# hangxu0304/DeepReduce

Measured on NVIDIA H100. Metric: ResNet-50 images/sec (whole job, device-timed, max over ranks), higher is better.
Workload: dtype bf16

## Files before the change

deepreduce_b200/ops/csrc/bn.cu:

```cuda
#include <cuda_bf16.h>

#include <algorithm>

#include "common.cuh"
#include "ops.h"

namespace dr {

namespace {

constexpr int kVec = 8;
constexpr int kApplyThreads = 256;
constexpr int kReduceThreads = 128;

struct ChanParams {
  float m[kVec], inv[kVec], w[kVec], b[kVec];
};

__device__ __forceinline__ void load8(const float* __restrict__ p, float* d) {
  const float4 a = __ldg(reinterpret_cast<const float4*>(p));
  const float4 b = __ldg(reinterpret_cast<const float4*>(p) + 1);
  d[0] = a.x; d[1] = a.y; d[2] = a.z; d[3] = a.w;
  d[4] = b.x; d[5] = b.y; d[6] = b.z; d[7] = b.w;
}
// ... 145 lines not shown
  q.sh = h - 2 * ph + 1;
  q.sw = w - 2 * pw + 1;
  q.off = ((n * pg.Ho + ph) * pg.Wo + pw) * C + c;
#pragma unroll
  for (int k = 0; k < 4; ++k) {
    const int a = k >> 1, b = k & 1;
    q.code[k] = a < q.nh && b < q.nw ? *reinterpret_cast<const uint2*>(codes + q.off + (a * pg.Wo + b) * C) : uint2{};
  }
}

template <bool kTwo>
__device__ __forceinline__ void pool_gather_grads(PoolGather& q, const __nv_bfloat16* __restrict__ gp,
                                                  const __nv_bfloat16* __restrict__ gp2, const PoolGeom& pg, int C) {
#pragma unroll
  for (int k = 0; k < 4; ++k) {
    const int a = k >> 1, b = k & 1;
    const bool in = a < q.nh && b < q.nw;
    const int off = q.off + (a * pg.Wo + b) * C;
    q.g[k] = in ? *reinterpret_cast<const uint4*>(gp + off) : uint4{};
    if (kTwo && in) q.g[k] = add_bf16x8(q.g[k], *reinterpret_cast<const uint4*>(gp2 + off));
  }
}

__device__ __forceinline__ void pool_gather_resolve(const PoolGather& q, uint4& g, unsigned& bits) {
  __nv_bfloat16* hg = reinterpret_cast<__nv_bfloat16*>(&g);
  const bool single = q.nh == 1 && q.nw == 1;
  bits = 0;
#pragma unroll
  for (int i = 0; i < kVec; ++i) {
    float s = 0.f;
    __nv_bfloat16 one = __float2bfloat16_rn(0.f);
    unsigned bit = 0;
#pragma unroll
    for (int k = 0; k < 4; ++k) {
      const int a = k >> 1, b = k & 1;
      const unsigned code = (reinterpret_cast<const uint8_t*>(&q.code[k]))[i];
      if (a < q.nh && b < q.nw && (int)(code & 0x7fu) == (q.sh - 2 * a) * 3 + (q.sw - 2 * b)) {
        const __nv_bfloat16 v = (reinterpret_cast<const __nv_bfloat16*>(&q.g[k]))[i];
        s = __fadd_rn(s, __bfloat162float(v));
        one = v;
        bit = code >> 7;
      }
    }
    hg[i] = single ? one : __float2bfloat16_rn(s);
    bits |= bit << i;
  }
}

template <bool kTwo>
__global__ void __launch_bounds__(kApplyThreads) bn_pool_grad_kernel(const __nv_bfloat16* __restrict__ gp,
                                                                     const __nv_bfloat16* __restrict__ gp2,
                                                                     const uint8_t* __restrict__ codes,
                                                                     __nv_bfloat16* __restrict__ g, PoolGeom pg,
                                                                     int64_t rows, int C) {
  const int groups = C / kVec;
  const int rows_per_cta = blockDim.x / groups;
  const int rsub = threadIdx.x / groups;
  if (rsub >= rows_per_cta) return;
  const int c = (threadIdx.x % groups) * kVec;
  const int64_t step = (int64_t)gridDim.x * rows_per_cta;
#pragma unroll 2
  for (int64_t r = (int64_t)blockIdx.x * rows_per_cta + rsub; r < rows; r += step) {
    PoolGather q;
    pool_gather_codes(q, codes, pg, (int)r, C, c, true);
    pool_gather_grads<kTwo>(q, gp, gp2, pg, C);
    uint4 v;
    unsigned bits;
    pool_gather_resolve(q, v, bits);
    __nv_bfloat16* hv = reinterpret_cast<__nv_bfloat16*>(&v);
#pragma unroll
    for (int i = 0; i < kVec; ++i)
      if (!((bits >> i) & 1u)) hv[i] = __float2bfloat16_rn(0.f);
    *reinterpret_cast<uint4*>(g + r * C + c) = v;
  }
}

struct RowTree {
  int block_y, grid_y;
  __host__ __device__ int S() const { return block_y * grid_y; }
  __host__ __device__ int loops(int rows) const { return 1 + (rows - 1) / (S() * kLoads); }
  static constexpr int kLoads = 4;
};

constexpr int kStatsThreads = 256;

__device__ __forceinline__ void welford_update(float x, float inv, float valid, float& mean, float& m2n) {
  const float d0 = __fsub_rn(x, mean);
  mean = __fmaf_rn(d0, inv, mean);
  const float d1 = __fsub_rn(x, mean);
  m2n = __fmaf_rn(__fmul_rn(d0, d1), valid, m2n);
}

template <int kN, bool kFuseNew>
__device__ __forceinline__ void welford_merge(int& n, float* mean, float* m2n, int n_new, const float* mean_new,
                                              const float* m2n_new) {
  const float fn = (float)n, fn_new = (float)n_new;
  const float factor = __frcp_rn((float)max(1, n + n_new));
#pragma unroll
  for (int i = 0; i < kN; ++i) {
    const float d = __fsub_rn(mean[i], mean_new[i]);
    const float s = kFuseNew ? __fmaf_rn(mean_new[i], fn_new, __fmul_rn(mean[i], fn))
                             : __fmaf_rn(mean[i], fn, __fmul_rn(mean_new[i], fn_new));
    mean[i] = __fmul_rn(s, factor);
    const float u = __fmul_rn(__fmul_rn(__fmul_rn(d, d), fn_new), fn);
    m2n[i] = __fadd_rn(m2n[i], __fmaf_rn(u, factor, m2n_new[i]));
  }
  n += n_new;
}

template <int kN>
struct WelfordSlots {
  float* mean; float* m2n; int* count;
  __device__ WelfordSlots(float* sh, int slots)
      : mean(sh), m2n(sh + slots * kN), count(reinterpret_cast<int*>(sh + 2 * slots * kN)) {}
  __device__ void put(int s, int n, const float* m, const float* q) const {
#pragma unroll
    for (int i = 0; i < kN; ++i) { mean[s * kN + i] = m[i]; m2n[s * kN + i] = q[i]; }
    count[s] = n;
  }
  template <bool kFuseNew>
  __device__ void merge_from(int s, int& n, float* m, float* q) const {
    float mn[kN], qn[kN];
#pragma unroll
    for (int i = 0; i < kN; ++i) { mn[i] = mean[s * kN + i]; qn[i] = m2n[s * kN + i]; }
    welford_merge<kN, kFuseNew>(n, m, q, count[s], mn, qn);
  }
  static size_t bytes(int slots) { return (size_t)slots * (2 * kN * sizeof(float) + sizeof(int)); }
};

template <int kN>
__device__ __forceinline__ void welford_tree_over_y(const WelfordSlots<kN>& sl, bool part, int y, int block_y, int base,
                                                    int stride, int& n, float* mean, float* m2n) {
  for (int off = block_y / 2; off > 0; off >>= 1) {
    if (part && y < 2 * off) sl.put(base + y * stride, n, mean, m2n);
    __syncthreads();
    if (part && y < off) sl.template merge_from<false>(base + (y + off) * stride, n, mean, m2n);
    __syncthreads();
  }
}

struct StatsOut {
  float* mean; float* invstd; float* running_mean; float* running_var;
  float* st_mean; float* st_m2n; int* st_count;
  float momentum, bessel, eps;
};

__device__ __forceinline__ void stats_store(const StatsOut& o, int c, int n, float mean, float m2n) {
  const float var = __fdiv_rn(m2n, (float)n);
  const float keep = __fsub_rn(1.f, o.momentum);
  o.mean[c] = mean;
  o.invstd[c] = rsqrtf(__fadd_rn(var, o.eps));
  o.running_mean[c] = __fmaf_rn(mean, o.momentum, __fmul_rn(o.running_mean[c], keep));
  o.running_var[c] = __fmaf_rn(__fmul_rn(var, o.bessel), o.momentum, __fmul_rn(o.running_var[c], keep));
}

__global__ void __launch_bounds__(kStatsThreads) bn_stats_kernel(const __nv_bfloat16* __restrict__ x, StatsOut o,
                                                                 RowTree t, int rows, int C) {
  constexpr int L = RowTree::kLoads;
  constexpr int kAhead = 4;
  extern __shared__ float sh[];
  const int gpc = blockDim.x / (L * t.block_y);
  const int g = threadIdx.x % gpc, j = (threadIdx.x / gpc) % L, y = threadIdx.x / (gpc * L);
  const int group = blockIdx.x * gpc + g;
  const bool live = group * kVec < C;
  const int c = live ? group * kVec : 0;
  const int S = t.S();
  const int n_loops = t.loops(rows);
  const int r0 = blockIdx.y * t.block_y + y + j * S;
  const int rstep = L * S;
  float mean[kVec], m2n[kVec];
#pragma unroll
  for (int i = 0; i < kVec; ++i) mean[i] = m2n[i] = 0.f;
  int n = 0;
  auto load = [&](uint4* b, int i0) {
#pragma unroll
    for (int u = 0; u < kAhead; ++u) {
      const int r = r0 + (i0 + u) * rstep;
      b[u] = live && i0 + u < n_loops && r < rows ? *reinterpret_cast<const uint4*>(x + (size_t)r * C + c) : uint4{};
    }
  };
  uint4 cur[kAhead];
  load(cur, 0);
  for (int i0 = 0; i0 < n_loops; i0 += kAhead) {
    uint4 nxt[kAhead];
    load(nxt, i0 + kAhead);
#pragma unroll
    for (int u = 0; u < kAhead; ++u) {
      const int i = i0 + u;
      if (i >= n_loops) break;
      const bool valid = r0 + i * rstep < rows;
      const float inv = valid ? __frcp_rn((float)(i + 1)) : 0.f;
      const float fv = valid ? 1.f : 0.f;
      n += valid;
      const __nv_bfloat16* hx = reinterpret_cast<const __nv_bfloat16*>(&cur[u]);
#pragma unroll
      for (int k = 0; k < kVec; ++k) welford_update(__bfloat162float(hx[k]), inv, fv, mean[k], m2n[k]);
    }
#pragma unroll
    for (int u = 0; u < kAhead; ++u) cur[u] = nxt[u];
  }
  const WelfordSlots<kVec> sl(sh, blockDim.x);
  sl.put(threadIdx.x, n, mean, m2n);
  __syncthreads();
  if (j == 0) {
#pragma unroll
    for (int a = 1; a < L; ++a) sl.merge_from<true>(threadIdx.x + a * gpc, n, mean, m2n);
  }
  __syncthreads();
  welford_tree_over_y<kVec>(sl, j == 0, y, t.block_y, g, gpc * L, n, mean, m2n);
  if (j != 0 || y != 0 || !live) return;
  if (t.grid_y == 1) {
#pragma unroll
    for (int i = 0; i < kVec; ++i) stats_store(o, c + i, n, mean[i], m2n[i]);
    return;
  }
#pragma unroll
  for (int i = 0; i < kVec; ++i) {
    o.st_mean[(size_t)blockIdx.y * C + c + i] = mean[i];
    o.st_m2n[(size_t)blockIdx.y * C + c + i] = m2n[i];
  }
  if (group == 0) o.st_count[blockIdx.y] = n;
}

__global__ void bn_stats_finalize_kernel(StatsOut o, RowTree t, int C) {
  extern __shared__ float sh[];
  const int cols = blockDim.x / t.block_y;
  const int col = threadIdx.x % cols, y = threadIdx.x / cols;
  const int c = blockIdx.x * cols + col;
  int n = 0;
  float mean = 0.f, m2n = 0.f;
  if (c < C)
    for (int b = y; b < t.grid_y; b += t.block_y) {
      const float mb = o.st_mean[(size_t)b * C + c], qb = o.st_m2n[(size_t)b * C + c];
      welford_merge<1, false>(n, &mean, &m2n, o.st_count[b], &mb, &qb);
    }
  const WelfordSlots<1> sl(sh, blockDim.x);
  welford_tree_over_y<1>(sl, true, y, t.block_y, col, cols, n, &mean, &m2n);
  if (y == 0 && c < C) stats_store(o, c, n, mean, m2n);
}


template <int kN>
__device__ __forceinline__ void tree_over_y(float* v, float* sh, int y, int n, int col, int width) {
  for (int off = n / 2; off > 0; off >>= 1) {
#pragma unroll
    for (int i = 0; i < kN; ++i) sh[y * width + col + i] = v[i];
    __syncthreads();
    if (y < off) {
#pragma unroll
      for (int i = 0; i < kN; ++i) v[i] = __fadd_rn(v[i], sh[(y + off) * width + col + i]);
    }
    __syncthreads();
  }
}

struct BwdOut {
  float* sums;
  float* dw; float* db; float* dwz; float* dbz;
  float* staging;
};

__device__ __forceinline__ void bwd_store(const BwdOut& o, int k, int c, int C, float v, const float* invstd,
                                         const float* invstd_z) {
  o.sums[k * C + c] = v;
  if (k == 0) {
    o.db[c] = v;
    if (o.dbz) o.dbz[c] = v;
  } else if (k == 1) {
    o.dw[c] = __fmul_rn(v, invstd[c]);
  } else {
    o.dwz[c] = __fmul_rn(v, invstd_z[c]);
  }
}

__device__ __forceinline__ float masked(__nv_bfloat16 go, unsigned bit) { return bit ? __bfloat162float(go) : 0.f; }

template <int kMode, bool kTwo>
__global__ void __launch_bounds__(kReduceThreads) bn_bwd_reduce_kernel(const __nv_bfloat16* __restrict__ go,
                                                                       const __nv_bfloat16* __restrict__ go2,
                                                                       const uint8_t* __restrict__ mask,
                                                                       const __nv_bfloat16* __restrict__ x,
                                                                       const float* __restrict__ mean,
                                                                       const float* __restrict__ invstd,
                                                                       const __nv_bfloat16* __restrict__ z,
                                                                       const float* __restrict__ mean_z,
                                                                       const float* __restrict__ invstd_z,
                                                                       __nv_bfloat16* __restrict__ g_out, BwdOut o,
                                                                       RowTree t, int rows, int C) {
  constexpr int kSums = kMode == 2 ? 3 : 2;
  constexpr int L = RowTree::kLoads;
  extern __shared__ float sh[];
  const int gpc = blockDim.x / t.block_y;
  const int tg = threadIdx.x % gpc, y = threadIdx.x / gpc;
  const int group = blockIdx.x * gpc + tg;
  const bool live = group * kVec < C;
  const int c = live ? group * kVec : 0;
  const int S = t.S();
  float m[kVec], mz[kVec];
#pragma unroll
  for (int i = 0; i < kVec; ++i) {
    m[i] = mean[c + i];
    mz[i] = kMode == 2 ? mean_z[c + i] : 0.f;
  }
  float acc[kSums][L][kVec];
#pragma unroll
  for (int k = 0; k < kSums; ++k)
#pragma unroll
    for (int j = 0; j < L; ++j)
#pragma unroll
      for (int i = 0; i < kVec; ++i) acc[k][j][i] = 0.f;
  const int mgroups = C / kVec;
  int r = blockIdx.y * t.block_y + y;
  const int n_loops = t.loops(rows);
  constexpr bool kAhead = !(kTwo && kMode == 2);
  struct Batch {
    uint4 g[L], g2[L], x[L], z[L];
    unsigned m[L];
  };
  auto load = [&](Batch& b, int r0) {
#pragma unroll
    for (int j = 0; j < L; ++j) {
// ... 186 lines not shown
  bn_apply_kernel<kMode><<<grid, threads, 0, st>>>(reinterpret_cast<const __nv_bfloat16*>(x), px,
                                                   reinterpret_cast<const __nv_bfloat16*>(z), pz,
                                                   reinterpret_cast<__nv_bfloat16*>(out),
                                                   reinterpret_cast<uint8_t*>(mask), rows, C);
  return cudaGetLastError();
}

int last_pow2(unsigned n) {
  n |= n >> 1; n |= n >> 2; n |= n >> 4; n |= n >> 8; n |= n >> 16;
  return std::max<int>(1, (int)(n - (n >> 1)));
}

RowTree row_tree(int rows, int C) {
  const int block_x = std::min(last_pow2((unsigned)C), 32);
  const int block_y = std::min(last_pow2((unsigned)((rows + 15) / 16)), 512 / block_x);
  int grid_y = std::min((rows + block_y * 16 - 1) / (block_y * 16), 128);
  if (grid_y < 8) grid_y = 1;
  return {block_y, grid_y};
}

template <int kMode, bool kTwo>
cudaError_t launch_bwd_reduce(const BnBwd& b, const RowTree& t, const BwdOut& o, int rows, int C, cudaStream_t st) {
  const int groups = C / kVec;
  const int gpc = std::min(groups, std::max(1, kReduceThreads / t.block_y));
  const dim3 grid((groups + gpc - 1) / gpc, t.grid_y);
  const int threads = gpc * t.block_y;
  count_launch();
  bn_bwd_reduce_kernel<kMode, kTwo><<<grid, threads, threads * kVec * sizeof(float), st>>>(
      reinterpret_cast<const __nv_bfloat16*>(b.go), reinterpret_cast<const __nv_bfloat16*>(b.go2), b.mask,
      reinterpret_cast<const __nv_bfloat16*>(b.x), b.px.mean, b.px.invstd, reinterpret_cast<const __nv_bfloat16*>(b.z),
      b.pz.mean, b.pz.invstd, reinterpret_cast<__nv_bfloat16*>(b.g), o, t, rows, C);
  return cudaGetLastError();
}

template <int kMode, bool kTwo>
cudaError_t launch_bwd_elemt(const BnBwd& b, const ElemtArgs& a, int64_t rows, int C, cudaStream_t st) {
  int grid = 0, threads = 0;
  cudaError_t e = rows_grid(bn_bwd_elemt_kernel<kMode, kTwo>, rows, C, grid, threads);
  if (e != cudaSuccess) return e;
  const float norm = (float)(1.0 / (double)rows);
  count_launch();
  bn_bwd_elemt_kernel<kMode, kTwo><<<grid, threads, 0, st>>>(
      reinterpret_cast<const __nv_bfloat16*>(kMode == 1 || kMode == 3 ? b.g : b.go),
      reinterpret_cast<const __nv_bfloat16*>(b.go2), b.mask, reinterpret_cast<const __nv_bfloat16*>(b.x),
      reinterpret_cast<const __nv_bfloat16*>(b.z), a, reinterpret_cast<__nv_bfloat16*>(b.dx),
      reinterpret_cast<__nv_bfloat16*>(b.dz), norm, rows, C);
  return cudaGetLastError();
}

template <int kMode, bool kTwo>
cudaError_t launch_backward(const BnBwd& b, int64_t rows64, int C, cudaStream_t st) {
  const int rows = (int)rows64;
  const RowTree t = row_tree(rows, C);
  const BwdOut o{b.sums, b.dw, b.db, b.dwz, b.dbz, b.staging};
  cudaError_t e;
  if (kMode == 3) {
    int grid = 0, threads = 0;
    e = rows_grid(bn_pool_grad_kernel<kTwo>, rows64, C, grid, threads);
    if (e != cudaSuccess) return e;
    count_launch();
    bn_pool_grad_kernel<kTwo><<<grid, threads, 0, st>>>(reinterpret_cast<const __nv_bfloat16*>(b.go),
                                                        reinterpret_cast<const __nv_bfloat16*>(b.go2), b.mask,
                                                        reinterpret_cast<__nv_bfloat16*>(b.g), b.pool, rows64, C);
    e = cudaGetLastError();
    if (e != cudaSuccess) return e;
  }
  BnBwd bb = b;
  if (kMode == 3) bb.go = b.g;
  e = launch_bwd_reduce<kMode, kTwo && kMode != 3>(bb, t, o, rows, C, st);
  if (e != cudaSuccess) return e;
  if (t.grid_y > 1) {
    const int cols = std::max(1, 512 / t.block_y);
    const int threads = cols * t.block_y;
    count_launch();
    bn_bwd_finalize_kernel<<<(C + cols - 1) / cols, threads, threads * sizeof(float), st>>>(
        o, t, kMode == 2 ? 3 : 2, C, b.px.invstd, b.pz.invstd);
    e = cudaGetLastError();
    if (e != cudaSuccess) return e;
  }
  const ElemtArgs a{b.px.mean, b.px.invstd, b.px.weight, b.sums, b.pz.mean, b.pz.invstd, b.pz.weight};
  return launch_bwd_elemt<kMode, kTwo && kMode == 2>(b, a, rows64, C, st);
}

cudaError_t launch_stats(const BnStats& s, int rows, int C, cudaStream_t st) {
  const RowTree t = row_tree(rows, C);
  const int grid_y = t.grid_y;
  const StatsOut o{s.mean, s.invstd, s.running_mean, s.running_var,
                   s.staging, s.staging + (size_t)grid_y * C, reinterpret_cast<int*>(s.staging + 2 * (size_t)grid_y * C),
                   s.momentum, s.bessel, s.eps};
  const int groups = C / kVec;
  const int gpc = std::min(groups, std::max(1, kStatsThreads / (RowTree::kLoads * t.block_y)));
  const int threads = gpc * RowTree::kLoads * t.block_y;
  count_launch();
  bn_stats_kernel<<<dim3((groups + gpc - 1) / gpc, grid_y), threads, WelfordSlots<kVec>::bytes(threads), st>>>(
      reinterpret_cast<const __nv_bfloat16*>(s.x), o, t, rows, C);
  cudaError_t e = cudaGetLastError();
  if (e != cudaSuccess || grid_y == 1) return e;
  const int cols = std::max(1, 512 / t.block_y);
  const int fthreads = cols * t.block_y;
  count_launch();
  bn_stats_finalize_kernel<<<(C + cols - 1) / cols, fthreads, WelfordSlots<1>::bytes(fthreads), st>>>(o, t, C);
  return cudaGetLastError();
}

}

void bn_row_tree(int64_t rows, int C, int* block_y, int* grid_y) {
  const RowTree t = row_tree((int)rows, C);
  *block_y = t.block_y;
  *grid_y = t.grid_y;
}

cudaError_t launch_bn_backward(int mode, const BnBwd& b, int64_t rows, int C, cudaStream_t st) {
  if (rows == 0) return cudaSuccess;
  const bool two = b.go2 != nullptr;
  switch (mode) {
    case 0: return two ? cudaErrorInvalidValue : launch_backward<0, false>(b, rows, C, st);
    case 1: return two ? launch_backward<1, true>(b, rows, C, st) : launch_backward<1, false>(b, rows, C, st);
    case 2: return two ? launch_backward<2, true>(b, rows, C, st) : launch_backward<2, false>(b, rows, C, st);
    case 3: return two ? launch_backward<3, true>(b, rows, C, st) : launch_backward<3, false>(b, rows, C, st);
    default: return cudaErrorInvalidValue;
  }
}

cudaError_t launch_bn_stats(const BnStats& s, int64_t rows, int C, cudaStream_t st) {
  if (rows == 0) return cudaSuccess;
  return launch_stats(s, (int)rows, C, st);
}

cudaError_t launch_bn_update_stats(const float* mean, float* var_invstd, float* running_mean, float* running_var, int C,
                                   float momentum, float bessel, float eps, cudaStream_t st) {
  count_launch();
  bn_update_stats_kernel<<<(C + 255) / 256, 256, 0, st>>>(mean, var_invstd, running_mean, running_var, C, momentum,
                                                          bessel, eps);
  return cudaGetLastError();
}

cudaError_t launch_bn_apply(int mode, const void* x, const BnParams& px, const void* z, const BnParams& pz, void* out,
                            void* mask, int64_t rows, int C, cudaStream_t st) {
  switch (mode) {
    case 0: return launch_apply<0>(x, px, z, pz, out, mask, rows, C, st);
    case 1: return launch_apply<1>(x, px, z, pz, out, mask, rows, C, st);
    case 2: return launch_apply<2>(x, px, z, pz, out, mask, rows, C, st);
    default: return cudaErrorInvalidValue;
  }
}

cudaError_t launch_bn_apply_pool(const void* x, const BnParams& px, void* out, void* codes, int N, const PoolGeom& pg,
                                 int C, cudaStream_t st) {
  const int64_t orows = (int64_t)N * pg.Ho * pg.Wo;
  if (orows == 0) return cudaSuccess;
  int grid = 0, threads = 0;
  cudaError_t e = rows_grid(bn_apply_pool_kernel, orows, C, grid, threads);
  if (e != cudaSuccess) return e;
  count_launch();
  bn_apply_pool_kernel<<<grid, threads, 0, st>>>(reinterpret_cast<const __nv_bfloat16*>(x), px,
                                                 reinterpret_cast<__nv_bfloat16*>(out),
                                                 reinterpret_cast<uint8_t*>(codes), orows, pg, C);
  return cudaGetLastError();
}

}
```

deepreduce_b200/ops/csrc/binding.cpp:

```cpp
#include <ATen/cuda/CUDAContext.h>
#include <c10/cuda/CUDAGuard.h>
#include <c10/cuda/CUDAStream.h>
#include <torch/extension.h>

#include <algorithm>
#include <condition_variable>
#include <deque>
#include <mutex>
#include <thread>

#include "ops.h"

namespace py = pybind11;
using dr::EngineParams;

#define CHECK_CUDA_T(x) TORCH_CHECK((x).is_cuda() && (x).is_contiguous(), #x " must be a contiguous CUDA tensor")

static cudaStream_t cur_stream() { return at::cuda::getCurrentCUDAStream().stream(); }

static void check_last(const char* what) {
  cudaError_t e = cudaGetLastError();
  TORCH_CHECK(e == cudaSuccess, what, ": ", cudaGetErrorString(e));
}

// ... 237 lines not shown
                  ") lies outside the DDP buffer of ", ddp_numel, " elements");
      TORCH_CHECK(e >= 0 && e % V == 0, "Repack: segment ", i, " starts at engine element ", e,
                  ", not on a 16-byte vector");
      TORCH_CHECK((e + n + V - 1) / V * V <= eng_numel, "Repack: segment ", i, " [", e, ", ", e + n,
                  ") lies outside the engine buffer of ", eng_numel, " elements");
      h[4 * i] = d; h[4 * i + 1] = e; h[4 * i + 2] = n; h[4 * i + 3] = n_vec;
      n_vec += (n + V - 1) / V;
      ddp_ranges.emplace_back(d, d + n);
      eng_ranges.emplace_back(e, e + n);
    }
    h[4 * n_seg] = 0; h[4 * n_seg + 1] = 0; h[4 * n_seg + 2] = 0; h[4 * n_seg + 3] = n_vec;
    for (auto* r : {&ddp_ranges, &eng_ranges}) {
      std::sort(r->begin(), r->end());
      for (size_t i = 1; i < r->size(); ++i)
        TORCH_CHECK((*r)[i].first >= (*r)[i - 1].second, "Repack: segments overlap at element ", (*r)[i].first);
    }
    table = host.to(device);
  }

  void check_buffers(const torch::Tensor& ddp, const torch::Tensor& eng) const {
    for (const torch::Tensor* t : {&ddp, &eng}) {
      TORCH_CHECK(t->is_cuda() && t->is_contiguous() && t->dim() == 1, "Repack: buffers are contiguous 1-D CUDA tensors");
      TORCH_CHECK(t->scalar_type() == dtype, "Repack: the table was built for ", dtype, " buffers, got ", t->scalar_type());
      TORCH_CHECK(t->device() == table.device(), "Repack: buffer on ", t->device(), ", table on ", table.device());
    }
    TORCH_CHECK(ddp.numel() >= ddp_numel, "Repack: the DDP buffer has ", ddp.numel(), " elements, the table needs ", ddp_numel);
    TORCH_CHECK(eng.numel() >= eng_numel, "Repack: the engine buffer has ", eng.numel(), " elements, the table needs ", eng_numel);
    TORCH_CHECK(reinterpret_cast<uintptr_t>(eng.data_ptr()) % 16 == 0, "Repack: the engine buffer must be 16-byte aligned");
  }

  void pack(torch::Tensor ddp, torch::Tensor eng) const {
    check_buffers(ddp, eng);
    c10::cuda::CUDAGuard g(eng.device());
    cudaError_t e = dr::launch_bucket_repack(true, elem_bytes, ddp.data_ptr(), eng.data_ptr(), table.data_ptr<int64_t>(),
                                             (int)n_seg, n_vec, cur_stream());
    TORCH_CHECK(e == cudaSuccess, "bucket_pack: ", cudaGetErrorString(e));
  }

  void unpack(torch::Tensor eng, torch::Tensor ddp) const {
    check_buffers(ddp, eng);
    c10::cuda::CUDAGuard g(eng.device());
    cudaError_t e = dr::launch_bucket_repack(false, elem_bytes, eng.data_ptr(), ddp.data_ptr(), table.data_ptr<int64_t>(),
                                             (int)n_seg, n_vec, cur_stream());
    TORCH_CHECK(e == cudaSuccess, "bucket_unpack: ", cudaGetErrorString(e));
  }
};

namespace at::native {
struct Var;
template <typename scalar_t, typename VarTransform>
void batch_norm_stats_channels_last_cuda_template(const at::Tensor& out_mean, const at::Tensor& out_invstd,
                                                   const at::Tensor& input, double epsilon);
}

static void check_bn_input(const torch::Tensor& x) {
  TORCH_CHECK(x.is_cuda() && x.scalar_type() == torch::kBFloat16 && x.dim() == 4 && x.stride(1) == 1 &&
                  x.is_contiguous(at::MemoryFormat::ChannelsLast),
              "bn: x must be a channels_last bf16 CUDA tensor");
  TORCH_CHECK(x.size(1) % 8 == 0 && x.size(1) <= 8192, "bn: channels must be a multiple of 8, at most 8192");
  TORCH_CHECK(x.numel() < std::numeric_limits<int32_t>::max(), "bn: tensor too large for 32-bit indexing");
}

static void check_chan(const torch::Tensor& t, int64_t C, const char* what) {
  TORCH_CHECK(t.is_cuda() && t.scalar_type() == torch::kFloat32 && t.is_contiguous() && t.numel() == C, "bn: ", what,
              " must be a contiguous float32 CUDA tensor of C elements");
}

static std::vector<torch::Tensor> bn_stats(torch::Tensor x, torch::Tensor running_mean, torch::Tensor running_var,
                                           double momentum, double eps, bool torch_kernel) {
  check_bn_input(x);
  const int64_t C = x.size(1);
  check_chan(running_mean, C, "running_mean");
  check_chan(running_var, C, "running_var");
  const int64_t N = x.numel() / C;
  TORCH_CHECK(N > 1, "bn: expected more than 1 value per channel when training");
  c10::cuda::CUDAGuard g(x.device());
  auto opts = x.options().dtype(torch::kFloat32);
  auto mean = torch::empty({C}, opts), invstd = torch::empty({C}, opts);
  const float bessel = static_cast<float>(static_cast<double>(N) / static_cast<double>(N - 1));
  int block_y = 0, grid_y = 0;
  dr::bn_row_tree(N, (int)C, &block_y, &grid_y);
  cudaError_t e;
  if (!torch_kernel && (int64_t)block_y * grid_y <= N) {
    auto staging = grid_y > 1 ? torch::empty({(2 * C + 1) * grid_y}, opts) : torch::Tensor();
    const dr::BnStats s{x.data_ptr(), mean.data_ptr<float>(), invstd.data_ptr<float>(), running_mean.data_ptr<float>(),
                        running_var.data_ptr<float>(), grid_y > 1 ? staging.data_ptr<float>() : nullptr,
                        (float)momentum, bessel, (float)eps};
    e = dr::launch_bn_stats(s, N, (int)C, cur_stream());
  } else {
    at::native::batch_norm_stats_channels_last_cuda_template<c10::BFloat16, at::native::Var>(mean, invstd, x, eps);
    e = dr::launch_bn_update_stats(mean.data_ptr<float>(), invstd.data_ptr<float>(), running_mean.data_ptr<float>(),
                                   running_var.data_ptr<float>(), (int)C, (float)momentum, bessel, (float)eps,
                                   cur_stream());
  }
  TORCH_CHECK(e == cudaSuccess, "bn_stats: ", cudaGetErrorString(e));
  return {mean, invstd};
}

static dr::BnParams bn_params(const std::vector<torch::Tensor>& p, int64_t C) {
  TORCH_CHECK(p.size() == 4, "bn: expected (mean, invstd, weight, bias)");
  const char* names[4] = {"mean", "invstd", "weight", "bias"};
  for (int i = 0; i < 4; ++i) check_chan(p[i], C, names[i]);
  return {p[0].data_ptr<float>(), p[1].data_ptr<float>(), p[2].data_ptr<float>(), p[3].data_ptr<float>()};
}

static void check_like_x(const torch::Tensor& t, const torch::Tensor& x, const char* what) {
  TORCH_CHECK(t.sizes() == x.sizes() && t.strides() == x.strides() && t.scalar_type() == torch::kBFloat16 &&
                  t.device() == x.device(),
              "bn: ", what, " must match x in shape, layout, dtype and device");
}

static std::vector<torch::Tensor> bn_apply(int64_t mode, torch::Tensor x, std::vector<torch::Tensor> p,
                                           c10::optional<torch::Tensor> z, std::vector<torch::Tensor> pz) {
  check_bn_input(x);
  const int64_t C = x.size(1);
  const dr::BnParams px = bn_params(p, C);
  dr::BnParams pzz{};
  const void* zp = nullptr;
  if (mode != 0) {
    TORCH_CHECK(z.has_value(), "bn: mode ", mode, " needs z");
    check_like_x(*z, x, "z");
    zp = z->data_ptr();
    if (mode == 2) pzz = bn_params(pz, C);
  }
  c10::cuda::CUDAGuard g(x.device());
  const int64_t rows = x.numel() / C;
  auto out = torch::empty_like(x);
  auto mask = torch::empty({rows, C / 8}, x.options().dtype(torch::kUInt8));
  cudaError_t e = dr::launch_bn_apply((int)mode, x.data_ptr(), px, zp, pzz, out.data_ptr(), mask.data_ptr(), rows,
                                      (int)C, cur_stream());
  TORCH_CHECK(e == cudaSuccess, "bn_apply: ", cudaGetErrorString(e));
  return {out, mask};
}

static std::vector<torch::Tensor> bn_apply_pool(torch::Tensor x, std::vector<torch::Tensor> p, int64_t kernel_size,
                                                int64_t stride, int64_t padding, int64_t dilation, bool ceil_mode) {
  TORCH_CHECK(kernel_size == 3 && stride == 2 && padding == 1 && dilation == 1 && !ceil_mode,
              "bn_apply_pool: only kernel 3, stride 2, padding 1, dilation 1, floor mode");
  check_bn_input(x);
  const int64_t N = x.size(0), C = x.size(1), H = x.size(2), W = x.size(3);
  const dr::BnParams px = bn_params(p, C);
  c10::cuda::CUDAGuard g(x.device());
  const dr::PoolGeom pg{(int)H, (int)W, (int)((H - 1) / 2 + 1), (int)((W - 1) / 2 + 1)};
  auto out = torch::empty({N, C, pg.Ho, pg.Wo}, x.options().memory_format(at::MemoryFormat::ChannelsLast));
  auto codes = torch::empty({N * pg.Ho * pg.Wo, C}, x.options().dtype(torch::kUInt8));
  cudaError_t e = dr::launch_bn_apply_pool(x.data_ptr(), px, out.data_ptr(), codes.data_ptr(), (int)N, pg, (int)C,
                                           cur_stream());
  TORCH_CHECK(e == cudaSuccess, "bn_apply_pool: ", cudaGetErrorString(e));
  return {out, codes};
}

static dr::BnParams bn_bwd_params(const std::vector<torch::Tensor>& p, int64_t C) {
  TORCH_CHECK(p.size() == 3, "bn_backward: expected (mean, invstd, weight)");
  const char* names[3] = {"mean", "invstd", "weight"};
  for (int i = 0; i < 3; ++i) check_chan(p[i], C, names[i]);
  return {p[0].data_ptr<float>(), p[1].data_ptr<float>(), p[2].data_ptr<float>(), nullptr};
}

static std::vector<torch::Tensor> bn_backward(int64_t mode, torch::Tensor go, torch::Tensor mask, torch::Tensor x,
                                              std::vector<torch::Tensor> p, c10::optional<torch::Tensor> z,
                                              std::vector<torch::Tensor> pz, c10::optional<torch::Tensor> go2) {
  TORCH_CHECK(mode >= 0 && mode <= 3, "bn_backward: mode must be 0, 1, 2 or 3");
  TORCH_CHECK(!go2.has_value() || mode != 0, "bn_backward: mode 0 takes no go2");
  check_bn_input(x);
  const int64_t C = x.size(1), rows = x.numel() / C;
  dr::PoolGeom pg{(int)x.size(2), (int)x.size(3), (int)((x.size(2) - 1) / 2 + 1), (int)((x.size(3) - 1) / 2 + 1)};
  const std::vector<int64_t> go_shape =
// ... 383 lines not shown
```

Measured before the change: 6144.

## Keep per-thread Welford chains in registers for large BN stats reductions

```diff
diff --git a/deepreduce_b200/ops/csrc/bn.cu b/deepreduce_b200/ops/csrc/bn.cu
--- a/deepreduce_b200/ops/csrc/bn.cu
+++ b/deepreduce_b200/ops/csrc/bn.cu
@@ -252,6 +252,8 @@
 };
 
 constexpr int kStatsThreads = 256;
+constexpr int kFinalizeThreads = 128;
+constexpr int kStatsRegsMinThreads = 32768;
 
 __device__ __forceinline__ void welford_update(float x, float inv, float valid, float& mean, float& m2n) {
   const float d0 = __fsub_rn(x, mean);
@@ -323,13 +325,17 @@
   o.running_var[c] = __fmaf_rn(__fmul_rn(var, o.bessel), o.momentum, __fmul_rn(o.running_var[c], keep));
 }
 
+template <bool kRegs>
 __global__ void __launch_bounds__(kStatsThreads) bn_stats_kernel(const __nv_bfloat16* __restrict__ x, StatsOut o,
                                                                  RowTree t, int rows, int C) {
   constexpr int L = RowTree::kLoads;
-  constexpr int kAhead = 4;
+  constexpr int kChains = kRegs ? L : 1;
+  constexpr int kPerY = L / kChains;
+  constexpr int kAhead = L / kChains;
   extern __shared__ float sh[];
-  const int gpc = blockDim.x / (L * t.block_y);
-  const int g = threadIdx.x % gpc, j = (threadIdx.x / gpc) % L, y = threadIdx.x / (gpc * L);
+  const int gpc = blockDim.x / (kPerY * t.block_y);
+  const int g = threadIdx.x % gpc, j = kRegs ? 0 : (threadIdx.x / gpc) % L, y = threadIdx.x / (gpc * kPerY);
+  const bool lead = j == 0;
   const int group = blockIdx.x * gpc + g;
   const bool live = group * kVec < C;
   const int c = live ? group * kVec : 0;
@@ -337,61 +343,81 @@
   const int n_loops = t.loops(rows);
   const int r0 = blockIdx.y * t.block_y + y + j * S;
   const int rstep = L * S;
-  float mean[kVec], m2n[kVec];
-#pragma unroll
-  for (int i = 0; i < kVec; ++i) mean[i] = m2n[i] = 0.f;
-  int n = 0;
+  float mean[kChains][kVec], m2n[kChains][kVec];
+  int n[kChains];
+#pragma unroll
+  for (int k = 0; k < kChains; ++k) {
+    n[k] = 0;
+#pragma unroll
+    for (int i = 0; i < kVec; ++i) mean[k][i] = m2n[k][i] = 0.f;
+  }
   auto load = [&](uint4* b, int i0) {
 #pragma unroll
-    for (int u = 0; u < kAhead; ++u) {
-      const int r = r0 + (i0 + u) * rstep;
-      b[u] = live && i0 + u < n_loops && r < rows ? *reinterpret_cast<const uint4*>(x + (size_t)r * C + c) : uint4{};
-    }
+    for (int u = 0; u < kAhead; ++u)
+#pragma unroll
+      for (int k = 0; k < kChains; ++k) {
+        const int r = r0 + (i0 + u) * rstep + k * S;
+        b[u * kChains + k] =
+            live && i0 + u < n_loops && r < rows ? *reinterpret_cast<const uint4*>(x + (size_t)r * C + c) : uint4{};
+      }
   };
-  uint4 cur[kAhead];
+  uint4 cur[L];
   load(cur, 0);
   for (int i0 = 0; i0 < n_loops; i0 += kAhead) {
-    uint4 nxt[kAhead];
+    uint4 nxt[L];
     load(nxt, i0 + kAhead);
 #pragma unroll
     for (int u = 0; u < kAhead; ++u) {
       const int i = i0 + u;
       if (i >= n_loops) break;
-      const bool valid = r0 + i * rstep < rows;
-      const float inv = valid ? __frcp_rn((float)(i + 1)) : 0.f;
-      const float fv = valid ? 1.f : 0.f;
-      n += valid;
-      const __nv_bfloat16* hx = reinterpret_cast<const __nv_bfloat16*>(&cur[u]);
-#pragma unroll
-      for (int k = 0; k < kVec; ++k) welford_update(__bfloat162float(hx[k]), inv, fv, mean[k], m2n[k]);
-    }
-#pragma unroll
-    for (int u = 0; u < kAhead; ++u) cur[u] = nxt[u];
+      const float rinv = __frcp_rn((float)(i + 1));
+#pragma unroll
+      for (int k = 0; k < kChains; ++k) {
+        const bool valid = r0 + i * rstep + k * S < rows;
+        const float inv = valid ? rinv : 0.f;
+        const float fv = valid ? 1.f : 0.f;
+        n[k] += valid;
+        const __nv_bfloat16* hx = reinterpret_cast<const __nv_bfloat16*>(&cur[u * kChains + k]);
+#pragma unroll
+        for (int e = 0; e < kVec; ++e) welford_update(__bfloat162float(hx[e]), inv, fv, mean[k][e], m2n[k][e]);
+      }
+    }
+#pragma unroll
+    for (int u = 0; u < L; ++u) cur[u] = nxt[u];
   }
   const WelfordSlots<kVec> sl(sh, blockDim.x);
-  sl.put(threadIdx.x, n, mean, m2n);
-  __syncthreads();
-  if (j == 0) {
-#pragma unroll
-    for (int a = 1; a < L; ++a) sl.merge_from<true>(threadIdx.x + a * gpc, n, mean, m2n);
-  }
-  __syncthreads();
-  welford_tree_over_y<kVec>(sl, j == 0, y, t.block_y, g, gpc * L, n, mean, m2n);
-  if (j != 0 || y != 0 || !live) return;
+  float* const m = mean[0];
+  float* const q = m2n[0];
+  int& cnt = n[0];
+  if (kRegs) {
+#pragma unroll
+    for (int a = 1; a < kChains; ++a) welford_merge<kVec, true>(cnt, m, q, n[a], mean[a], m2n[a]);
+  } else {
+    sl.put(threadIdx.x, cnt, m, q);
+    __syncthreads();
+    if (lead) {
+#pragma unroll
+      for (int a = 1; a < L; ++a) sl.merge_from<true>(threadIdx.x + a * gpc, cnt, m, q);
+    }
+    __syncthreads();
+  }
+  welford_tree_over_y<kVec>(sl, lead, y, t.block_y, g, gpc * kPerY, cnt, m, q);
+  if (!lead || y != 0 || !live) return;
   if (t.grid_y == 1) {
 #pragma unroll
-    for (int i = 0; i < kVec; ++i) stats_store(o, c + i, n, mean[i], m2n[i]);
+    for (int i = 0; i < kVec; ++i) stats_store(o, c + i, cnt, m[i], q[i]);
     return;
   }
 #pragma unroll
   for (int i = 0; i < kVec; ++i) {
-    o.st_mean[(size_t)blockIdx.y * C + c + i] = mean[i];
-    o.st_m2n[(size_t)blockIdx.y * C + c + i] = m2n[i];
-  }
-  if (group == 0) o.st_count[blockIdx.y] = n;
-}
-
-__global__ void bn_stats_finalize_kernel(StatsOut o, RowTree t, int C) {
+    o.st_mean[(size_t)blockIdx.y * C + c + i] = m[i];
+    o.st_m2n[(size_t)blockIdx.y * C + c + i] = q[i];
+  }
+  if (group == 0) o.st_count[blockIdx.y] = cnt;
+}
+
+__global__ void __launch_bounds__(kFinalizeThreads) bn_stats_finalize_kernel(StatsOut o, RowTree t, int C) {
+  constexpr int kRows = 8;
   extern __shared__ float sh[];
   const int cols = blockDim.x / t.block_y;
   const int col = threadIdx.x % cols, y = threadIdx.x / cols;
@@ -399,9 +425,20 @@
   int n = 0;
   float mean = 0.f, m2n = 0.f;
   if (c < C)
-    for (int b = y; b < t.grid_y; b += t.block_y) {
-      const float mb = o.st_mean[(size_t)b * C + c], qb = o.st_m2n[(size_t)b * C + c];
-      welford_merge<1, false>(n, &mean, &m2n, o.st_count[b], &mb, &qb);
+    for (int b0 = y; b0 < t.grid_y; b0 += kRows * t.block_y) {
+      float mb[kRows], qb[kRows];
+      int nb[kRows];
+#pragma unroll
+      for (int k = 0; k < kRows; ++k) {
+        const int b = b0 + k * t.block_y;
+        const bool in = b < t.grid_y;
+        mb[k] = in ? o.st_mean[(size_t)b * C + c] : 0.f;
+        qb[k] = in ? o.st_m2n[(size_t)b * C + c] : 0.f;
+        nb[k] = in ? o.st_count[b] : 0;
+      }
+#pragma unroll
+      for (int k = 0; k < kRows; ++k)
+        if (b0 + k * t.block_y < t.grid_y) welford_merge<1, false>(n, &mean, &m2n, nb[k], &mb[k], &qb[k]);
     }
   const WelfordSlots<1> sl(sh, blockDim.x);
   welford_tree_over_y<1>(sl, true, y, t.block_y, col, cols, n, &mean, &m2n);
@@ -758,25 +795,32 @@
   return launch_bwd_elemt<kMode, kTwo && kMode == 2>(b, a, rows64, C, st);
 }
 
-cudaError_t launch_stats(const BnStats& s, int rows, int C, cudaStream_t st) {
-  const RowTree t = row_tree(rows, C);
+template <bool kRegs>
+cudaError_t launch_stats(const BnStats& s, const RowTree& t, int rows, int C, cudaStream_t st) {
   const int grid_y = t.grid_y;
   const StatsOut o{s.mean, s.invstd, s.running_mean, s.running_var,
                    s.staging, s.staging + (size_t)grid_y * C, reinterpret_cast<int*>(s.staging + 2 * (size_t)grid_y * C),
                    s.momentum, s.bessel, s.eps};
+  const int per_y = kRegs ? 1 : RowTree::kLoads;
   const int groups = C / kVec;
-  const int gpc = std::min(groups, std::max(1, kStatsThreads / (RowTree::kLoads * t.block_y)));
-  const int threads = gpc * RowTree::kLoads * t.block_y;
+  const int gpc = std::min(groups, std::max(1, kStatsThreads / (per_y * t.block_y)));
+  const int threads = gpc * per_y * t.block_y;
   count_launch();
-  bn_stats_kernel<<<dim3((groups + gpc - 1) / gpc, grid_y), threads, WelfordSlots<kVec>::bytes(threads), st>>>(
+  bn_stats_kernel<kRegs><<<dim3((groups + gpc - 1) / gpc, grid_y), threads, WelfordSlots<kVec>::bytes(threads), st>>>(
       reinterpret_cast<const __nv_bfloat16*>(s.x), o, t, rows, C);
   cudaError_t e = cudaGetLastError();
   if (e != cudaSuccess || grid_y == 1) return e;
-  const int cols = std::max(1, 512 / t.block_y);
+  const int cols = std::max(1, kFinalizeThreads / t.block_y);
   const int fthreads = cols * t.block_y;
   count_launch();
   bn_stats_finalize_kernel<<<(C + cols - 1) / cols, fthreads, WelfordSlots<1>::bytes(fthreads), st>>>(o, t, C);
   return cudaGetLastError();
+}
+
+cudaError_t launch_stats(const BnStats& s, int rows, int C, cudaStream_t st) {
+  const RowTree t = row_tree(rows, C);
+  return (int64_t)t.S() * (C / kVec) >= kStatsRegsMinThreads ? launch_stats<true>(s, t, rows, C, st)
+                                                             : launch_stats<false>(s, t, rows, C, st);
 }
 
 }
```

Result: faster. 6266, median of 6 (+2.0%).

## Fuse BN stats finalize into stats kernel via last-block ticket reduction

Applied to the files above, without the earlier changes.

```diff
diff --git a/deepreduce_b200/ops/csrc/binding.cpp b/deepreduce_b200/ops/csrc/binding.cpp
--- a/deepreduce_b200/ops/csrc/binding.cpp
+++ b/deepreduce_b200/ops/csrc/binding.cpp
@@ -343,7 +343,7 @@
   dr::bn_row_tree(N, (int)C, &block_y, &grid_y);
   cudaError_t e;
   if (!torch_kernel && (int64_t)block_y * grid_y <= N) {
-    auto staging = grid_y > 1 ? torch::empty({(2 * C + 1) * grid_y}, opts) : torch::Tensor();
+    auto staging = grid_y > 1 ? torch::empty({2 * C * grid_y}, opts) : torch::Tensor();
     const dr::BnStats s{x.data_ptr(), mean.data_ptr<float>(), invstd.data_ptr<float>(), running_mean.data_ptr<float>(),
                         running_var.data_ptr<float>(), grid_y > 1 ? staging.data_ptr<float>() : nullptr,
                         (float)momentum, bessel, (float)eps};
diff --git a/deepreduce_b200/ops/csrc/bn.cu b/deepreduce_b200/ops/csrc/bn.cu
--- a/deepreduce_b200/ops/csrc/bn.cu
+++ b/deepreduce_b200/ops/csrc/bn.cu
@@ -251,7 +251,8 @@
   static constexpr int kLoads = 4;
 };
 
-constexpr int kStatsThreads = 256;
+constexpr int kStatsThreadsPerSm = 1024;
+constexpr int kStatsLongChain = 16;
 
 __device__ __forceinline__ void welford_update(float x, float inv, float valid, float& mean, float& m2n) {
   const float d0 = __fsub_rn(x, mean);
@@ -310,7 +311,7 @@
 
 struct StatsOut {
   float* mean; float* invstd; float* running_mean; float* running_var;
-  float* st_mean; float* st_m2n; int* st_count;
+  float* st_mean; float* st_m2n;
   float momentum, bessel, eps;
 };
 
@@ -323,11 +324,16 @@
   o.running_var[c] = __fmaf_rn(__fmul_rn(var, o.bessel), o.momentum, __fmul_rn(o.running_var[c], keep));
 }
 
-__global__ void __launch_bounds__(kStatsThreads) bn_stats_kernel(const __nv_bfloat16* __restrict__ x, StatsOut o,
-                                                                 RowTree t, int rows, int C) {
+constexpr int kStatsMaxColumns = 1024;
+__device__ unsigned g_stats_tickets[kStatsMaxColumns];
+
+template <int kThreads>
+__global__ void __launch_bounds__(kThreads, kStatsThreadsPerSm / kThreads)
+    bn_stats_kernel(const __nv_bfloat16* __restrict__ x, StatsOut o, RowTree t, int rows, int C) {
   constexpr int L = RowTree::kLoads;
-  constexpr int kAhead = 4;
+  constexpr int kRing = 4;
   extern __shared__ float sh[];
+  __shared__ bool last;
   const int gpc = blockDim.x / (L * t.block_y);
   const int g = threadIdx.x % gpc, j = (threadIdx.x / gpc) % L, y = threadIdx.x / (gpc * L);
   const int group = blockIdx.x * gpc + g;
@@ -341,32 +347,27 @@
 #pragma unroll
   for (int i = 0; i < kVec; ++i) mean[i] = m2n[i] = 0.f;
   int n = 0;
-  auto load = [&](uint4* b, int i0) {
-#pragma unroll
-    for (int u = 0; u < kAhead; ++u) {
-      const int r = r0 + (i0 + u) * rstep;
-      b[u] = live && i0 + u < n_loops && r < rows ? *reinterpret_cast<const uint4*>(x + (size_t)r * C + c) : uint4{};
-    }
+  auto load = [&](int i) {
+    const int r = r0 + i * rstep;
+    return live && r < rows ? *reinterpret_cast<const uint4*>(x + (size_t)r * C + c) : uint4{};
   };
-  uint4 cur[kAhead];
-  load(cur, 0);
-  for (int i0 = 0; i0 < n_loops; i0 += kAhead) {
-    uint4 nxt[kAhead];
-    load(nxt, i0 + kAhead);
-#pragma unroll
-    for (int u = 0; u < kAhead; ++u) {
+  uint4 ring[kRing];
+#pragma unroll
+  for (int u = 0; u < kRing; ++u) ring[u] = load(u);
+  for (int i0 = 0; i0 < n_loops; i0 += kRing) {
+#pragma unroll
+    for (int u = 0; u < kRing; ++u) {
       const int i = i0 + u;
       if (i >= n_loops) break;
       const bool valid = r0 + i * rstep < rows;
       const float inv = valid ? __frcp_rn((float)(i + 1)) : 0.f;
       const float fv = valid ? 1.f : 0.f;
       n += valid;
-      const __nv_bfloat16* hx = reinterpret_cast<const __nv_bfloat16*>(&cur[u]);
+      const __nv_bfloat16* hx = reinterpret_cast<const __nv_bfloat16*>(&ring[u]);
 #pragma unroll
       for (int k = 0; k < kVec; ++k) welford_update(__bfloat162float(hx[k]), inv, fv, mean[k], m2n[k]);
-    }
-#pragma unroll
-    for (int u = 0; u < kAhead; ++u) cur[u] = nxt[u];
+      ring[u] = load(i + kRing);
+    }
   }
   const WelfordSlots<kVec> sl(sh, blockDim.x);
   sl.put(threadIdx.x, n, mean, m2n);
@@ -377,35 +378,64 @@
   }
   __syncthreads();
   welford_tree_over_y<kVec>(sl, j == 0, y, t.block_y, g, gpc * L, n, mean, m2n);
-  if (j != 0 || y != 0 || !live) return;
+  const bool head = j == 0 && y == 0 && live;
   if (t.grid_y == 1) {
-#pragma unroll
-    for (int i = 0; i < kVec; ++i) stats_store(o, c + i, n, mean[i], m2n[i]);
+    if (head)
+#pragma unroll
+      for (int i = 0; i < kVec; ++i) stats_store(o, c + i, n, mean[i], m2n[i]);
     return;
   }
-#pragma unroll
-  for (int i = 0; i < kVec; ++i) {
-    o.st_mean[(size_t)blockIdx.y * C + c + i] = mean[i];
-    o.st_m2n[(size_t)blockIdx.y * C + c + i] = m2n[i];
-  }
-  if (group == 0) o.st_count[blockIdx.y] = n;
-}
-
-__global__ void bn_stats_finalize_kernel(StatsOut o, RowTree t, int C) {
-  extern __shared__ float sh[];
-  const int cols = blockDim.x / t.block_y;
-  const int col = threadIdx.x % cols, y = threadIdx.x / cols;
-  const int c = blockIdx.x * cols + col;
-  int n = 0;
-  float mean = 0.f, m2n = 0.f;
-  if (c < C)
-    for (int b = y; b < t.grid_y; b += t.block_y) {
-      const float mb = o.st_mean[(size_t)b * C + c], qb = o.st_m2n[(size_t)b * C + c];
-      welford_merge<1, false>(n, &mean, &m2n, o.st_count[b], &mb, &qb);
-    }
-  const WelfordSlots<1> sl(sh, blockDim.x);
-  welford_tree_over_y<1>(sl, true, y, t.block_y, col, cols, n, &mean, &m2n);
-  if (y == 0 && c < C) stats_store(o, c, n, mean, m2n);
+  if (head) {
+#pragma unroll
+    for (int i = 0; i < kVec; ++i) {
+      o.st_mean[(size_t)blockIdx.y * C + c + i] = mean[i];
+      o.st_m2n[(size_t)blockIdx.y * C + c + i] = m2n[i];
+    }
+    __threadfence();
+  }
+  __syncthreads();
+  if (threadIdx.x == 0) {
+    last = atomicAdd(&g_stats_tickets[blockIdx.x], 1u) == gridDim.y - 1;
+    if (last) g_stats_tickets[blockIdx.x] = 0;
+  }
+  __syncthreads();
+  if (!last) return;
+  constexpr int kF = kVec / L;
+  const int cols = gpc * L;
+  const int col = threadIdx.x % cols;
+  const int cf = blockIdx.x * gpc * kVec + col * kF;
+  const bool flive = cf < C;
+  const int full = rows / S, rem = rows % S;
+  int fn = 0;
+  float fm[kF], fq[kF];
+#pragma unroll
+  for (int i = 0; i < kF; ++i) fm[i] = fq[i] = 0.f;
+  constexpr int kPre = 4;
+  if (flive)
+    for (int b0 = y; b0 < t.grid_y; b0 += kPre * t.block_y) {
+      float mb[kPre][kF], qb[kPre][kF];
+#pragma unroll
+      for (int u = 0; u < kPre; ++u) {
+        const int b = b0 + u * t.block_y;
+#pragma unroll
+        for (int i = 0; i < kF; ++i) {
+          mb[u][i] = b < t.grid_y ? __ldcg(o.st_mean + (size_t)b * C + cf + i) : 0.f;
+          qb[u][i] = b < t.grid_y ? __ldcg(o.st_m2n + (size_t)b * C + cf + i) : 0.f;
+        }
+      }
+#pragma unroll
+      for (int u = 0; u < kPre; ++u) {
+        const int b = b0 + u * t.block_y;
+        if (b >= t.grid_y) break;
+        const int nb = t.block_y * full + min(max(rem - b * t.block_y, 0), t.block_y);
+        welford_merge<kF, false>(fn, fm, fq, nb, mb[u], qb[u]);
+      }
+    }
+  const WelfordSlots<kF> fsl(sh, blockDim.x);
+  welford_tree_over_y<kF>(fsl, true, y, t.block_y, col, cols, fn, fm, fq);
+  if (y == 0 && flive)
+#pragma unroll
+    for (int i = 0; i < kF; ++i) stats_store(o, cf + i, fn, fm[i], fq[i]);
 }
 
 
@@ -758,25 +788,25 @@
   return launch_bwd_elemt<kMode, kTwo && kMode == 2>(b, a, rows64, C, st);
 }
 
+template <int kThreads>
+cudaError_t launch_stats_sized(const StatsOut& o, const RowTree& t, const void* x, int rows, int C, cudaStream_t st) {
+  const int groups = C / kVec;
+  const int gpc = std::min(groups, std::max(1, kThreads / (RowTree::kLoads * t.block_y)));
+  const int threads = gpc * RowTree::kLoads * t.block_y;
+  const int columns = (groups + gpc - 1) / gpc;
+  if (t.grid_y > 1 && columns > kStatsMaxColumns) return cudaErrorInvalidValue;
+  count_launch();
+  bn_stats_kernel<kThreads><<<dim3(columns, t.grid_y), threads, WelfordSlots<kVec>::bytes(threads), st>>>(
+      reinterpret_cast<const __nv_bfloat16*>(x), o, t, rows, C);
+  return cudaGetLastError();
+}
+
 cudaError_t launch_stats(const BnStats& s, int rows, int C, cudaStream_t st) {
   const RowTree t = row_tree(rows, C);
-  const int grid_y = t.grid_y;
-  const StatsOut o{s.mean, s.invstd, s.running_mean, s.running_var,
-                   s.staging, s.staging + (size_t)grid_y * C, reinterpret_cast<int*>(s.staging + 2 * (size_t)grid_y * C),
+  const StatsOut o{s.mean, s.invstd, s.running_mean, s.running_var, s.staging, s.staging + (size_t)t.grid_y * C,
                    s.momentum, s.bessel, s.eps};
-  const int groups = C / kVec;
-  const int gpc = std::min(groups, std::max(1, kStatsThreads / (RowTree::kLoads * t.block_y)));
-  const int threads = gpc * RowTree::kLoads * t.block_y;
-  count_launch();
-  bn_stats_kernel<<<dim3((groups + gpc - 1) / gpc, grid_y), threads, WelfordSlots<kVec>::bytes(threads), st>>>(
-      reinterpret_cast<const __nv_bfloat16*>(s.x), o, t, rows, C);
-  cudaError_t e = cudaGetLastError();
-  if (e != cudaSuccess || grid_y == 1) return e;
-  const int cols = std::max(1, 512 / t.block_y);
-  const int fthreads = cols * t.block_y;
-  count_launch();
-  bn_stats_finalize_kernel<<<(C + cols - 1) / cols, fthreads, WelfordSlots<1>::bytes(fthreads), st>>>(o, t, C);
-  return cudaGetLastError();
+  const bool wide = t.loops(rows) >= kStatsLongChain && C / kVec >= 2 * (512 / (RowTree::kLoads * t.block_y));
+  return wide ? launch_stats_sized<512>(o, t, s.x, rows, C, st) : launch_stats_sized<256>(o, t, s.x, rows, C, st);
 }
 
 }
```

Result: faster. 6169 before, 6242 after, median of 6 (+1.2%).
